# mcbuehler/DeepSEE

Hardware: AMD Instinct MI355X
Metric: train-step images/sec (G+D fwd+bwd), 8x 32->256 bs=8 (higher is better)
Workload: dtype fp32

## Files before the change

deepsee_amd/ops.py:

```python
import os
import ctypes as C

import threading

import torch

from . import lib as L
from .plan import KernelPlan, DEFAULT_PLAN, current as P

LRELU_SLOPE = 0.2
BN_EPS = 1e-5
BN_MOMENTUM = 0.1
SN_EPS = 1e-12
NHIDDEN = 128

_scratch = {}

PROFILE = None
PROFILE_BYTES = {}
PROFILE_OPERAND_GB = 0.0


def _variant(geom, modulate=False):
    halo = (geom.korder == 1 and geom.KH == 3 and geom.KW == 3 and geom.mul == 1 and geom.Hi == geom.Ho
# ... 1199 lines not shown
            dw = new(c)
            L.call("channel_dot_rng", dy, dw, C.c_long(m), c, ws, C.c_uint64(ctx.philox.seed),
                   C.c_uint64(ctx.philox.offset))
        elif eps is not None and ctx.needs_input_grad[1]:
            dw = channel_dot(dy, eps, c).clone()
        return dx, dw, None, None, None


class SeanInput(torch.autograd.Function):

    @staticmethod
    def forward(ctx, w_sh, b_sh, style, labels, shift, want_actv, want_style):
        n, h, w, nc = labels.n, labels.h, labels.w, labels.nc
        r, rw = h >> shift, w >> shift
        ld = (NHIDDEN if want_actv else 0) + (style.shape[2] if want_style else 0)
        cat = new(n, r, rw, ld)
        coff = 0
        if want_actv:
            table = new(9, nc, NHIDDEN)
            L.call("onehot_conv3x3_pack", w_sh.contiguous(), table, NHIDDEN, nc)
            L.call("onehot_conv3x3_fwd", labels.t, table, b_sh, cat, n, h, w, shift, nc, NHIDDEN, ld, 0, 1, -1, None, 0.0)
            coff = NHIDDEN
        if want_style:
            L.call("label_gather", labels.t, style.contiguous(), cat, n, h, w, shift, nc, style.shape[2], ld, coff, 1.0)
        ctx.labels, ctx.shift, ctx.want_actv, ctx.want_style, ctx.coff = labels, shift, want_actv, want_style, coff
        ctx.sshape = style.shape if want_style else None
        ctx.save_for_backward(cat)
        return cat

    @staticmethod
    def backward(ctx, dcat):
        (cat,) = ctx.saved_tensors
        lab, shift = ctx.labels, ctx.shift
        dcat = dcat.contiguous()
        n, r, rw, ld = cat.shape
        dw = db = dstyle = None
        if ctx.want_actv and ctx.needs_input_grad[0]:
            dw, db = new(NHIDDEN, lab.nc, 3, 3), new(NHIDDEN)
            ws = scratch(L.lib().dsee_onehot_conv3x3_wgrad_workspace(n, lab.h, lab.w, shift, lab.nc), "ohw")
            L.call("onehot_conv3x3_wgrad", lab.t, dcat, ld, cat, ld, n, lab.h, lab.w, shift, lab.nc, dw, db, ws)
        if ctx.want_style and ctx.needs_input_grad[2]:
            s = ctx.sshape[2]
            dstyle = new(*ctx.sshape)
            ws = scratch(L.lib().dsee_label_segsum_workspace(n, lab.h, lab.w, shift, lab.nc, s), "seg")
            L.call("label_segsum", lab.t, dcat, ld, ctx.coff, dstyle, n, lab.h, lab.w, shift, lab.nc, s, 1.0, ws)
        return dw, db, dstyle, None, None, None, None


class StylePool(torch.autograd.Function):

    @staticmethod
    def forward(ctx, feat, labels, shift):
        n, hf, wf, c = feat.shape
        assert hf == labels.h >> shift
        out = new(n, labels.nc, c)
        ws = scratch(L.lib().dsee_label_segsum_workspace(n, labels.h, labels.w, shift, labels.nc, c), "seg")
        L.call("label_segsum", labels.t, feat, c, 0, out, n, labels.h, labels.w, shift, labels.nc, c,
               1.0 / (hf * wf), ws)
        ctx.labels, ctx.shift, ctx.fshape = labels, shift, feat.shape
        return out

    @staticmethod
    def backward(ctx, ds):
        lab = ctx.labels
        n, hf, wf, c = ctx.fshape
        df = new(*ctx.fshape)
        L.call("label_gather", lab.t, ds.contiguous(), df, n, lab.h, lab.w, ctx.shift, lab.nc, c, c, 0, 1.0 / (hf * wf))
        return df, None, None


_perm_cache = {}


def packed_perm(c, device):
    key = (c, str(device))
    if key not in _perm_cache:
        rows = (c + 63) // 64 * 128
        idx = torch.full((rows,), 2 * c, dtype=torch.long)
        for p in range(rows):
            b, rem = divmod(p, 128)
            w, rem = divmod(rem, 64)
            h, cc = divmod(rem, 32)
            ch = b * 64 + w * 32 + cc
            if ch < c:
                idx[p] = h * c + ch
        _perm_cache[key] = (idx.to(device), rows)
    return _perm_cache[key]


def pack_gamma_beta(w_gamma, w_beta, b_gamma, b_beta):
    c = w_gamma.shape[0]
    idx, rows = packed_perm(c, w_gamma.device)
    zw = torch.zeros((1,) + tuple(w_gamma.shape[1:]), dtype=w_gamma.dtype, device=w_gamma.device)
    zb = torch.zeros(1, dtype=w_gamma.dtype, device=w_gamma.device)
    w2 = torch.cat([w_gamma, w_beta, zw], 0).index_select(0, idx)
    b2 = torch.cat([b_gamma, b_beta, zb], 0).index_select(0, idx)
    return w2, b2


class SeanPack(torch.autograd.Function):

    @staticmethod
    def forward(ctx, mode, wg, wb, wsg, wsb, bg, bb, bsg, bsb, ag, ab, amax=None):
        ref = wg if wg is not None else wsg
        c = ref.shape[0]
        k = wg.shape[1] if wg is not None else 0
        sdim = wsg.shape[1] if wsg is not None else 0
        rows = L.lib().dsee_sean_pack_rows(c)
        w2a = new(rows, k, 3, 3) if mode != 2 else None
        wst = new(9 * rows, sdim) if mode in (1, 2) else None
        b2 = new(rows)
        L.call("sean_pack_fwd", wg, wb, wsg, wsb, bg, bb, bsg, bsb, ag, ab, int(mode), c, k, sdim, w2a, wst, b2, amax)
        ctx.mode, ctx.dims = int(mode), (c, k, sdim, rows)
        ctx.save_for_backward(wg, wb, wsg, wsb, bg, bb, bsg, bsb, ag, ab)
        return w2a, wst, b2

    @staticmethod
    def backward(ctx, dw2a, dwst, db2):
        wg, wb, wsg, wsb, bg, bb, bsg, bsb, ag, ab = ctx.saved_tensors
        c, k, sdim, rows = ctx.dims
        mode = ctx.mode
        if mode != 2 and dw2a is None:
            dw2a = torch.zeros(rows, k, 3, 3, dtype=torch.float32, device=db2.device if db2 is not None else wg.device)
        if mode in (1, 2) and dwst is None:
            dwst = torch.zeros(9 * rows, sdim, dtype=torch.float32, device=wsg.device)
        outs = [torch.empty_like(t) if (t is not None and ctx.needs_input_grad[i + 1]) else None
                for i, t in enumerate((wg, wb, wsg, wsb, bg, bb, bsg, bsb))]
        dalpha = new(2) if (mode in (1, 3) and (ctx.needs_input_grad[9] or ctx.needs_input_grad[10])) else None
        ws = scratch(L.lib().dsee_sean_pack_bwd_workspace(), "seanpack")
        L.call("sean_pack_bwd", wg, wb, wsg, wsb, bg, bb, bsg, bsb, ag, ab, mode, c, k, sdim,
               None if dw2a is None else dw2a.contiguous(), None if dwst is None else dwst.contiguous(),
               None if db2 is None else db2.contiguous(), *outs, dalpha, ws)
        da = (dalpha[0:1], dalpha[1:2]) if dalpha is not None else (None, None)
        return (None, *outs, da[0] if ctx.needs_input_grad[9] else None, da[1] if ctx.needs_input_grad[10] else None, None)


class TableLayout(torch.autograd.Function):

    @staticmethod
    def forward(ctx, t, n, nc, rows, amax=None):
        ctx.dims = (n, nc, rows)
        out = new(n, 9, rows, 32)
        L.call("style_table_layout", t.contiguous(), out, n, nc, rows, amax)
        return out

    @staticmethod
    def backward(ctx, dout):
        n, nc, rows = ctx.dims
        dt = new(n * nc, 9 * rows)
        L.call("style_table_layout_bwd", dout.contiguous(), dt, n, nc, rows)
        return dt, None, None, None, None


def style_table_packed(style, wst, rows, amax=None):
    n, nc, s = style.shape
    t = TableLayout.apply(_style_gemm(style.reshape(n * nc, s), wst), n, nc, rows, amax)
    t.dsee_amax = amax
    return t


class SyncBNConfig:

    def __init__(self, world, group=None, clamp=True):
        self.world, self.group, self.clamp = int(world), group, bool(clamp)


def _stats_rows_ok(c):
    return P().sync_bn is None and c % 4 == 0 and c // 4 <= 256 and 256 % (c // 4) == 0


def bn_stats(x, running_mean, running_var, training):
    n, h, w, c = x.shape
    mean, invstd = new(c), new(c)
    if not training:
        L.call("norm_eval_stats", running_mean, running_var, c, BN_EPS, mean, invstd)
        return mean, invstd, None
    cfg = P().sync_bn
    if cfg is None:
        rows = getattr(x, "dsee_stats_rows", None)
        if rows is not None:
            L.call("norm_stats_finalize_parts", rows[0], rows[1], c, BN_EPS, BN_MOMENTUM, mean, invstd, running_mean,
                   running_var)
            return mean, invstd, None
        part = getattr(x, "dsee_stats_part", None)
        if part is None:
            part = torch.empty(L.lib().dsee_norm_workspace(n, h * w, c, 1) // 4, dtype=torch.float32, device="cuda")
            L.call("norm_stats_partial", x, n, h * w, c, 1, part)
            if P().share_stats:
                x.dsee_stats_part = part
        L.call("norm_stats_finalize", part, n, h * w, c, 1, BN_EPS, BN_MOMENTUM, mean, invstd, running_mean, running_var)
        return mean, invstd, None
    ws = scratch(L.lib().dsee_norm_workspace(n, h * w, c, 1), "norm")
    from . import parallel
    local = new(2, c)
    L.call("norm_stats_local", x, n, h * w, c, local, ws)
    rows = parallel.gather_stats(local, cfg.world, cfg.group)
    L.call("norm_stats_merge", rows, cfg.world, n * h * w, c, BN_EPS, BN_MOMENTUM, int(cfg.clamp), mean, invstd,
           running_mean, running_var)
    return mean, invstd, cfg


def in_stats(x):
    n, h, w, c = x.shape
    mean, invstd = new(n, c), new(n, c)
    part = getattr(x, "dsee_in_part", None)
    if part is None:
        part = torch.empty(L.lib().dsee_norm_workspace(n, h * w, c, n) // 4, dtype=torch.float32, device="cuda")
        L.call("norm_stats_partial", x, n, h * w, c, n, part)
        if P().share_stats:
            x.dsee_in_part = part
    L.call("norm_stats_finalize", part, n, h * w, c, n, BN_EPS, BN_MOMENTUM, mean, invstd, None, None)
    return mean, invstd


def norm_stats(x, running_mean, running_var, training):
    if running_mean is None:
        mean, invstd = in_stats(x)
        return mean, invstd, None
    return bn_stats(x, running_mean, running_var, training)


def stat_groups(mean):
    return mean.shape[0] if mean.dim() == 2 else 1


def _call_sg(name, sg, head, tail):
    if sg == 1:
        L.call(name, *head, *tail)
    else:
        L.call(name + "_sg", *head, sg, *tail)


def _wino_ws(n, h, w, c, sg):
    return (L.lib().dsee_modulate_bwd_wino_workspace(n, h, w, c) if sg == 1
            else L.lib().dsee_modulate_bwd_wino_workspace_sg(n, h, w, c, sg))


def modulate_bwd(dh, out, x, scale, mean, invstd, rows, cfg, as_dm=False, add=None, xhat_amax=None, mask=None):
    n, h, w, c = x.shape
    sg = stat_groups(mean)
    dx = torch.empty_like(x)
    sums = new(2 * sg + 2, c)
    dgb = dm = None
    t = n * (h // 4) * (w // 4)
    dha = carried_amax(dh)
    pre = (as_dm and P().presplit_dm and P().presplit_gb and xhat_amax is not None and dha is not None and t % 256 == 0
           and sg == 1)
    s16 = scale.dtype == torch.float16
    if s16 and not (pre and P().half):
        scale, s16 = scale.float(), False
    if pre:
        ga = amax_slot()
        L.call("amax_product", dha, xhat_amax, 1.0, ga)
        pk = P().half
        dm = (_i16(36 * t * rows * (1 if pk else 2)), ga, "pk" if pk else True)
        ws = scratch(L.lib().dsee_modulate_bwd_wino_workspace(n, h, w, c), "norm")
        L.call("modulate_bwd_reduce_wino_f16p" if pk else "modulate_bwd_reduce_wino_f16x2", dh.contiguous(),
               None if mask is not None else out, x, scale, mean, invstd, dm[0], rows, sums, n, h, w, c, LRELU_SLOPE, ws, ga,
               DM_BOUND, mask)
    elif as_dm:
        dm = (new(36, t, rows), amax_slot() if (P().gemm_split and (P().gemm_f16x2 or P().half)) else None)
        ws = scratch(_wino_ws(n, h, w, c, sg), "norm")
        _call_sg("modulate_bwd_reduce_wino", sg, (dh.contiguous(), out, x, scale, mean, invstd, dm[0], rows, sums, n, h, w, c),
                 (LRELU_SLOPE, ws, dm[1]))
    else:
        dgb = (torch.zeros if c % 64 else torch.empty)(n, h, w, rows, dtype=torch.float32, device=x.device)
        ws = scratch(L.lib().dsee_norm_workspace(n, h * w, c, sg), "norm")
        _call_sg("modulate_bwd_reduce", sg, (dh.contiguous(), out, x, scale, mean, invstd, dgb, rows, sums, n, h * w, c),
                 (LRELU_SLOPE, ws))
    count = (n // sg) * h * w
    if cfg is not None:
        from . import parallel
        parallel.allreduce_sums(sums[0:2], cfg.world, cfg.group)
        count *= cfg.world
    da = amax_slot()
    _call_sg("modulate_bwd_apply_amax", sg,
             (dh.contiguous(), None if mask is not None else out, x, scale, mean, invstd, sums, add, dx, n, h * w, c),
             (1.0 / count, LRELU_SLOPE, da, int(s16), mask))
    tag_amax(dx, da)
    return dx, dgb, sums[2 * sg:2 * sg + 2], dm


class SpadeNormAct(torch.autograd.Function):

    @staticmethod
    def forward(ctx, x, cat, w2, b2, running_mean, running_var, training, add_one, cat_ups, grad_sink=None):
        ctx.plan = P()
        ctx.grad_sink = grad_sink
        n, h, w, c = x.shape
        rows, kin = w2.shape[0], w2.shape[1]
        assert cat.shape[3] == kin and kin % 4 == 0
        mean, invstd, ctx.sync = norm_stats(x, running_mean, running_var, training)
        geom = L.geom_fwd(n, cat.shape[1], cat.shape[2], kin, rows, 3, 1, 1, cat_ups)
        assert geom.Ho == h and geom.Wo == w
        w2 = w2.contiguous()
        out, scale = torch.empty_like(x), torch.empty_like(x)
        wp = _pack_fwd(w2, kin, geom.korder)
        with _timed(_variant(geom, True), _flops(geom)):
            _call_sg("conv2d_modulate_fwd", stat_groups(mean),
                     (C.byref(geom), cat, wp, None, 0, b2.contiguous(), x, mean, invstd, out, scale, c),
                     (float(add_one), LRELU_SLOPE))
        ctx.geom = geom
        ctx.save_for_backward(x, cat, w2, out, scale, mean, invstd)
        return out

    @staticmethod
    @_under_plan
    def backward(ctx, dh):
        x, cat, w2, out, scale, mean, invstd = ctx.saved_tensors
# ... 402 lines not shown
```

deepsee_amd/plan.py:

```python
import contextlib
import dataclasses
import threading
from typing import Any, Optional


@dataclasses.dataclass(frozen=True)
class KernelPlan:
    winograd: bool = True
    winograd_wgrad: bool = True
    winograd_mod: bool = True
    gemm_split: bool = True
    gemm_af32: bool = True
    keep_v: bool = True
    gemm_f16x2: bool = True
    half: bool = False
    half_norms: bool = True
    presplit_a: bool = True
    gemm_w4: bool = True
    dgrad_s2_parity: bool = True
    presplit_min_tiles: int = 512
    conv_halo_f16: bool = True
    onehot_wgrad_mfma: bool = True
    conv_amax_out: bool = True
    presplit_dm: bool = True
    presplit_gb: bool = True
    dout_sums: bool = True
    adjoint_dgrad: bool = True
    fuse_noise: bool = True
    thin_gemm: bool = True
    share_stats: bool = True
    producer_stats: bool = True
    fuse_dm: bool = True
    fused_norm: bool = True
    fused_w4: bool = False
    sign_mask: bool = True
    defer_act: bool = True
    branch_streams: bool = False
    conv_f16x2_min_flop: float = 1e9
    sync_bn: Optional[Any] = None

    def replace(self, **changes):
        return dataclasses.replace(self, **changes)

    @contextlib.contextmanager
    def active(self):
        prev = getattr(_tls, "plan", None)
        _tls.plan = self
        try:
            yield self
        finally:
            _tls.plan = prev

    @classmethod
    def fields(cls):
        return [f.name for f in dataclasses.fields(cls)]


def _env_overrides():
    import ast
    import os
    text = os.environ.get("DSEE_PLAN", "").strip()
    if not text:
        return {}
    out = {}
    for item in text.split(","):
        k, _, v = item.partition("=")
        k = k.strip()
        if k not in KernelPlan.fields():
            raise ValueError("DSEE_PLAN: unknown KernelPlan field %r (fields: %s)" % (k, ", ".join(KernelPlan.fields())))
        out[k] = ast.literal_eval(v.strip())
    return out


DEFAULT_PLAN = KernelPlan(**_env_overrides())
_tls = threading.local()


def current():
    return getattr(_tls, "plan", None) or DEFAULT_PLAN


def from_opt(opt):
    prec = getattr(opt, "precision", "fp32")
    if prec not in ("fp32", "fp16"):
        raise ValueError("opt.precision must be 'fp32' or 'fp16', got %r" % (prec,))
    over = getattr(opt, "kernel_plan", None)
    if isinstance(over, KernelPlan):
        plan = over
    else:
        plan = DEFAULT_PLAN.replace(**dict(over or {}))
    return plan.replace(half=(prec == "fp16"))
```

include/deepsee_hip.h:

```cpp
#ifndef DEEPSEE_HIP_H
#define DEEPSEE_HIP_H

#include <stddef.h>
#include <stdint.h>

#ifdef __cplusplus
extern "C" {
#endif

#ifndef __HIP_INCLUDE_HIP_HIP_RUNTIME_API_H__
typedef struct ihipStream_t* hipStream_t;
#endif

#define DSEE_OK 0
#define DSEE_EINVAL (-1)
#define DSEE_ELAUNCH (-2)
#define DSEE_EUNSUPPORTED (-3)

#define DSEE_ACT_NONE 0
#define DSEE_ACT_LRELU 1
#define DSEE_ACT_RELU 2
#define DSEE_ACT_TANH 3
#define DSEE_ACT_MASK 4

// ... 195 lines not shown
int dsee_norm_eval_stats(const float* running_mean, const float* running_var, int C, float eps, float* mean,
                         float* invstd, hipStream_t stream);
int dsee_norm_act_fwd(const float* x, const float* mean, const float* invstd, float* y, int N, int HW, int C,
                      int groups, int act, float slope, hipStream_t stream);
int dsee_norm_act_bwd(const float* dy, const float* y, const float* x, const float* mean, const float* invstd,
                      float* dx, int N, int HW, int C, int groups, int act, float slope, float* workspace,
                      hipStream_t stream);
int dsee_norm_act_fwd_amax(const float* x, const float* mean, const float* invstd, float* y, int N, int HW, int C,
                           int groups, int act, float slope, float* amax_y, hipStream_t stream);
int dsee_norm_act_bwd_amax(const float* dy, const float* y, const float* x, const float* mean, const float* invstd,
                           float* dx, int N, int HW, int C, int groups, int act, float slope, float* workspace,
                           float* amax_dx, hipStream_t stream);
int dsee_bn_act_fwd(const float* x, const float* mean, const float* invstd, const float* gamma, const float* beta, float* y,
                    int N, int HW, int C, int act, float slope, float* amax_y, hipStream_t stream);
int dsee_bn_act_bwd_reduce(const float* dy, const float* y, const float* x, const float* mean, const float* invstd, int N,
                           int HW, int C, int act, float slope, float* sums, float* workspace, hipStream_t stream);
int dsee_bn_act_bwd_apply(const float* dy, const float* y, const float* x, const float* mean, const float* invstd,
                          const float* gamma, const float* sums, const float* local_sums, float inv_count, float* dx,
                          float* dgamma, float* dbeta, int N, int HW, int C, int act, float slope, float* amax_dx,
                          hipStream_t stream);
int dsee_counter_inc(int64_t* counter, hipStream_t stream);
int dsee_modulate_bwd(const float* dh, const float* h, const float* x, const float* scale, const float* mean,
                      const float* invstd, const float* add, float* dx, float* dgb, int dgb_ld, float* col_sums, int N,
                      int HW, int C, float slope, float* workspace, hipStream_t stream);

int dsee_modulate_bwd_reduce(const float* dh, const float* h, const float* x, const float* scale, const float* mean,
                             const float* invstd, float* dgb, int dgb_ld, float* sums, int N, int HW, int C, float slope,
                             float* workspace, hipStream_t stream);
size_t dsee_modulate_bwd_wino_workspace(int N, int H, int W, int C);
int dsee_modulate_bwd_reduce_wino(const float* dh, const float* h, const float* x, const float* scale, const float* mean,
                                  const float* invstd, float* dM, int rows, float* sums, int N, int H, int W, int C,
                                  float slope, float* workspace, float* amax, hipStream_t stream);
int dsee_modulate_bwd_reduce_wino_f16x2(const float* dh, const float* h, const float* x, const float* scale,
                                        const float* mean, const float* invstd, void* dM2, int rows, float* sums, int N,
                                        int H, int W, int C, float slope, float* workspace, const float* amax_g, float bound,
                                        const uint32_t* sign_mask,
        hipStream_t stream);
int dsee_amax_product(const float* a, const float* b, float floor_b, float* out, hipStream_t stream);
int dsee_wino43_input_adjoint_amax(const float* dV, float* dx, int N, int H, int W, int C, float* amax_dx, hipStream_t stream);
int dsee_modulate_bwd_apply(const float* dh, const float* h, const float* x, const float* scale, const float* mean,
                            const float* invstd, const float* sums, const float* add, float* dx, int N, int HW, int C,
                            float inv_count, float slope, hipStream_t stream);
int dsee_modulate_bwd_apply_amax(const float* dh, const float* h, const float* x, const float* scale, const float* mean,
                                 const float* invstd, const float* sums, const float* add, float* dx, int N, int HW, int C,
                                 float inv_count, float slope, float* amax_dx, int scale_f16, const uint32_t* sign_mask,
        hipStream_t stream);

int dsee_spade_fused_fwd_sg(const void* V2, const void* U2, const float* amax_cat, float v_bound, const float* amax_u,
                            const float* bias_packed, const float* x, const float* mean, const float* invstd, float* out_h,
                            float* out_scale, int N, int H, int W, int C, int rows, int K, int groups, int stat_groups,
                            float add_one, float slope, float* amax_h, float* amax_xhat, uint32_t* sign_mask,
                            hipStream_t stream);
int dsee_spade_fused_fwd_f16p_sg(const void* V1, const void* U1, const float* amax_cat, float v_bound, const float* amax_u,
                                 const float* bias_packed, const float* x, const float* mean, const float* invstd,
                                 float* out_h, float* out_scale, int N, int H, int W, int C, int rows, int K, int groups,
                                 int stat_groups, float add_one, float slope, float* amax_h, float* amax_xhat,
                                 uint32_t* sign_mask, hipStream_t stream);
int dsee_wino43_output_modulate_sg(const float* M, const float* bias_packed, const float* x, const float* mean,
                                   const float* invstd, float* out_h, float* out_scale, int N, int H, int W, int C, int rows,
                                   int stat_groups, float add_one, float slope, const float* mscale, hipStream_t stream);
int dsee_conv2d_modulate_fwd_sg(const dsee_conv_geom* g, const float* in, const float* w_packed,
                                const float* style_table, int shared_cin, const float* bias_packed, const float* x,
                                const float* mean, const float* invstd, float* out_h, float* out_scale, int C,
                                int stat_groups, float add_one, float slope, hipStream_t stream);
int dsee_modulate_bwd_reduce_sg(const float* dh, const float* h, const float* x, const float* scale, const float* mean,
                                const float* invstd, float* dgb, int dgb_ld, float* sums, int N, int HW, int C,
                                int stat_groups, float slope, float* workspace, hipStream_t stream);
size_t dsee_modulate_bwd_wino_workspace_sg(int N, int H, int W, int C, int stat_groups);
int dsee_modulate_bwd_reduce_wino_sg(const float* dh, const float* h, const float* x, const float* scale,
                                     const float* mean, const float* invstd, float* dM, int rows, float* sums, int N, int H,
                                     int W, int C, int stat_groups, float slope, float* workspace, float* amax,
                                     hipStream_t stream);
int dsee_modulate_bwd_apply_amax_sg(const float* dh, const float* h, const float* x, const float* scale, const float* mean,
                                    const float* invstd, const float* sums, const float* add, float* dx, int N, int HW, int C,
                                    int stat_groups, float inv_count, float slope, float* amax_dx, int scale_f16,
                                    const uint32_t* sign_mask, hipStream_t stream);

int dsee_onehot_conv3x3_pack(const float* w_oihw, float* table, int Co, int L, hipStream_t stream);
int dsee_onehot_conv3x3_fwd(const uint8_t* lab, const float* table, const float* bias, float* out, int N, int H, int W,
                            int shift, int L, int Co, int out_ld, int coff, int relu, int onehot_coff, float* amax,
                            float amax_floor, hipStream_t stream);
size_t dsee_onehot_conv3x3_wgrad_workspace(int N, int H, int W, int shift, int L);
int dsee_onehot_conv3x3_wgrad(const uint8_t* lab, const float* dact, int dact_ld, const float* act, int act_ld, int N,
                              int H, int W, int shift, int L, float* dw_oihw, float* dbias, float* workspace,
                              hipStream_t stream);
int dsee_label_onehot(const uint8_t* lab, float* out, int N, int H, int W, int shift, int out_ld, int coff,
                      hipStream_t stream);
int dsee_label_gather(const uint8_t* lab, const float* table, float* out, int N, int H, int W, int shift, int L, int Cs,
                      int out_ld, int coff, float scale, hipStream_t stream);
size_t dsee_label_segsum_workspace(int N, int H, int W, int shift, int L, int Cs);
int dsee_label_segsum(const uint8_t* lab, const float* in, int ld, int coff, float* table, int N, int H, int W,
                      int shift, int L, int Cs, float scale, float* workspace, hipStream_t stream);

int dsee_upsample_noise_fwd(const float* x, const float* eps, const float* noise_w, float* y, int N, int H, int W, int C,
                            int ups, hipStream_t stream);
int dsee_upsample_noise_rng_fwd(const float* x, const float* noise_w, float* y, int N, int H, int W, int C, int ups,
                                uint64_t seed, uint64_t offset, hipStream_t stream);
int dsee_upsample_noise_rng_fwd_stats(const float* x, const float* noise_w, float* y, int N, int H, int W, int C, int ups,
                                      uint64_t seed, uint64_t offset, float* stats_part, hipStream_t stream);
int dsee_channel_dot_rng(const float* a, float* out, long M, int C, float* workspace, uint64_t seed, uint64_t offset,
                         hipStream_t stream);
int dsee_sumpool(const float* dy, float* dx, int N, int H, int W, int C, int ups, hipStream_t stream);
int dsee_sumpool_amax(const float* dy, float* dx, int N, int H, int W, int C, int ups, float* amax_dx, hipStream_t stream);
size_t dsee_sumpool_dot_rng_workspace(int N, int H, int W, int C, int ups);
int dsee_sumpool_dot_rng(const float* dy, float* dx, int N, int H, int W, int C, int ups, float* amax_dx, float* dnoise_w,
                         float* workspace, uint64_t seed, uint64_t offset, hipStream_t stream);
size_t dsee_channel_dot_workspace(long M, int C);
int dsee_channel_dot(const float* a, const float* b, float* out, long M, int C, float* workspace, hipStream_t stream);
int dsee_act_fwd(const float* x, float* y, long n, int act, float slope, hipStream_t stream);
int dsee_act_bwd(const float* dy, const float* y, float* dx, long n, int act, float slope, hipStream_t stream);
int dsee_act_bwd_amax(const float* dy, const float* y, float* dx, long n, int act, float slope, float* amax_dx,
                      hipStream_t stream);
int dsee_axpby(const float* a, float alpha, const float* b, float beta, float* y, long n, hipStream_t stream);
int dsee_avgpool3s2_fwd(const float* x, float* y, int N, int H, int W, int C, hipStream_t stream);
int dsee_avgpool3s2_bwd(const float* dy, float* dx, int N, int H, int W, int C, hipStream_t stream);
int dsee_maxpool2_fwd(const float* x, float* y, int N, int H, int W, int C, hipStream_t stream);
int dsee_maxpool2_bwd(const float* dy, const float* x, float* dx, int N, int H, int W, int C, hipStream_t stream);
int dsee_nchw_to_nhwc(const float* x, float* y, int N, int C, int H, int W, int Cs, hipStream_t stream);
int dsee_nhwc_to_nchw(const float* x, float* y, int N, int C, int H, int W, int Cs, hipStream_t stream);
int dsee_label_to_u8(const float* label, uint8_t* out, long n, hipStream_t stream);
int dsee_bicubic_down(const float* x, float* y, int N, int H, int W, int S, int cs_in, int cs_out, hipStream_t stream);
int dsee_image_u8_to_nhwc(const uint8_t* img, const uint8_t* flip, float* out, int N, int H, int W, int cs_out,
                          hipStream_t stream);
int dsee_label_u8_prepare(const uint8_t* lab, const uint8_t* flip, uint8_t* out, int N, int H, int W, int unknown_to,
                          hipStream_t stream);
int dsee_build_d_input(const uint8_t* lab, const float* img, float* out, long pixels, int L, int Cs, int img_cs,
                       hipStream_t stream);
int dsee_build_d_input_amax(const uint8_t* lab, const float* img, float* out, long pixels, int L, int Cs, int img_cs,
                            float* amax_out, hipStream_t stream);
int dsee_extract_image_grad(const float* din, float* dimg, long pixels, int L, int Cs, int img_cs, hipStream_t stream);
int dsee_rng_fill(float* out, long n, uint64_t seed, uint64_t offset, int normal, hipStream_t stream);
int dsee_rng_set_epoch(const uint64_t* epoch_dev);

size_t dsee_loss_workspace(void);
int dsee_loss_fwd_bwd(int mode, const float* a, const float* b, float* grad, long rows, int ld, int valid_c,
                      float weight, float* loss_out, float* workspace, hipStream_t stream);
int dsee_loss_bwd(int mode, const float* a, const float* b, float* grad, long rows, int ld, int valid_c, float weight,
                  const float* upstream, hipStream_t stream);

int dsee_sean_pack_rows(int C);
int dsee_sean_pack_fwd(const float* w_gamma, const float* w_beta, const float* ws_gamma, const float* ws_beta,
                       const float* b_gamma, const float* b_beta, const float* bs_gamma, const float* bs_beta,
                       const float* alpha_gamma, const float* alpha_beta, int mode, int C, int K, int S, float* w2a,
                       float* wst, float* b2, float* amax_w2a, hipStream_t stream);
size_t dsee_sean_pack_bwd_workspace(void);
int dsee_sean_pack_bwd(const float* w_gamma, const float* w_beta, const float* ws_gamma, const float* ws_beta,
                       const float* b_gamma, const float* b_beta, const float* bs_gamma, const float* bs_beta,
                       const float* alpha_gamma, const float* alpha_beta, int mode, int C, int K, int S,
                       const float* dw2a, const float* dwst, const float* db2, float* dw_gamma, float* dw_beta,
                       float* dws_gamma, float* dws_beta, float* db_gamma, float* db_beta, float* dbs_gamma,
                       float* dbs_beta, float* dalpha, float* workspace, hipStream_t stream);
int dsee_style_table_layout(const float* t, float* table, int N, int L, int rows, float* amax, hipStream_t stream);
int dsee_style_table_layout_bwd(const float* dtable, float* dt, int N, int L, int rows, hipStream_t stream);

int dsee_spectral_norm_fwd(const float* w_orig, float* u, float* v, float* sigma, float* w_sn, int R, int K,
                           int power_iter, float eps, float* scratch, hipStream_t stream);
int dsee_spectral_norm_bwd(const float* dw, const float* w_sn, const float* u, const float* v, const float* sigma,
                           float* dw_orig, int R, int K, float* scratch, hipStream_t stream);

typedef struct dsee_sn_layer {
  const float* w_orig;
  float* u;
  float* v;
  int64_t out_off;
  int64_t saved_off;
  int32_t R, K;
  int32_t scratch_off;
  int32_t pad_;
} dsee_sn_layer;
int dsee_spectral_norm_group_fwd(const dsee_sn_layer* layers, int nlayers, const int* work_k, int n_k, const int* work_r,
                                 int n_r, const int* work_e, int n_e, int power_iter, float eps, float* scratch,
                                 float* sigma, float* out, float* saved, float* amax, hipStream_t stream);

typedef struct dsee_adam_tensor {
  int64_t offset;
  int64_t numel;
  int32_t first_block;
  int32_t step;
  float lr;
  int32_t active;
} dsee_adam_tensor;
int dsee_adam_step(float* param, const float* grad, float* exp_avg, float* exp_avg_sq,
                   const dsee_adam_tensor* tensors, const int* block_tensor, int nblocks, float beta1, float beta2,
                   float eps, float grad_scale, float clip, hipStream_t stream);
int dsee_grad_gather(const int64_t* grad_ptrs, const dsee_adam_tensor* tensors, const int* block_tensor, int nblocks,
                     float* grad_flat, int* active, hipStream_t stream);
int dsee_adam_step_range(float* param, const float* grad, float* exp_avg, float* exp_avg_sq,
                         const dsee_adam_tensor* tensors, const int* block_tensor, int first_block, int nblocks,
                         float beta1, float beta2, float eps, float grad_scale, float clip, hipStream_t stream);

#define DSEE_COMM_ID_BYTES 128
int dsee_comm_unique_id(void* id_out);
int dsee_comm_init(void** comm_out, const void* id, int world, int rank);
int dsee_comm_world(const void* comm);
int dsee_comm_rank(const void* comm);
int dsee_comm_allreduce_sum(void* comm, float* buf, long n, hipStream_t stream);
int dsee_comm_broadcast(void* comm, void* buf, long nbytes, int root, hipStream_t stream);
int dsee_comm_allgather(void* comm, const void* send, void* recv, long nbytes_per_rank, hipStream_t stream);
int dsee_comm_destroy(void* comm);

size_t dsee_sean_norm_fwd_workspace(int N, int H, int W, int C, int label_nc, int has_table);
int dsee_sean_norm_fwd(const uint8_t* labels, int lab_h, int lab_w, int shift, int label_nc, const float* w_shared,
                       const float* b_shared, const float* w2a, const float* table, const float* bias_packed, const float* x,
                       float* running_mean, float* running_var, int training, float eps, float momentum, float add_one,
                       float slope, float* out_h, float* out_scale, uint32_t* sign_mask, float* mean, float* invstd,
                       float* amax_h, int N, int H, int W, int C, void* workspace, size_t workspace_bytes,
                       hipStream_t stream);

typedef struct dsee_norm_layer {
  const float* w_shared;
  const float* b_shared;
  const float* w2a;
  const float* table;
  const float* bias_packed;
  float* running_mean;
  float* running_var;
  float add_one;
} dsee_norm_layer;
size_t dsee_spade_resblock_fwd_workspace(int N, int H, int W, int C, int label_nc, int has_table);
int dsee_spade_resblock_fwd(const dsee_norm_layer* norm_0, const float* w_conv_0, const float* b_conv_0,
                            const dsee_norm_layer* norm_1, const float* w_conv_1, const float* b_conv_1,
                            const uint8_t* labels, int lab_h, int lab_w, int shift, int label_nc, const float* x, float* out,
                            int out_act, int training, float eps, float momentum, float slope, int N, int H, int W, int C,
                            void* workspace, size_t workspace_bytes, hipStream_t stream);

typedef struct dsee_block_noise {
  const float* w_middle;
  uint64_t seed_middle, offset_middle;
  const float* w_skip;
  uint64_t seed_skip, offset_skip;
} dsee_block_noise;
typedef struct dsee_norm_grads {
  float* dw_shared;
  float* db_shared;
  float* dw2a;
  float* dtable;
  float* dgamma_beta_sums;
} dsee_norm_grads;
typedef struct dsee_block_grads {
  dsee_norm_grads norm_0, norm_1;
  float* dw_conv_0;
  float* db_conv_0;
  float* dw_conv_1;
  float* db_conv_1;
  float* dw_noise_middle;
  float* dw_noise_skip;
} dsee_block_grads;
size_t dsee_spade_resblock_saved_bytes(int N, int H, int W, int C, int label_nc, int has_table);
size_t dsee_spade_resblock_train_fwd_workspace(int N, int H, int W, int C, int label_nc, int has_table);
int dsee_spade_resblock_train_fwd(const dsee_norm_layer* norm_0, const float* w_conv_0, const float* b_conv_0,
                                  const dsee_norm_layer* norm_1, const float* w_conv_1, const float* b_conv_1,
                                  const dsee_block_noise* noise, const uint8_t* labels, int lab_h, int lab_w, int shift,
                                  int label_nc, const float* x, float* out, float eps, float momentum, float slope, int N, int H,
                                  int W, int C, void* saved, size_t saved_bytes, void* workspace, size_t workspace_bytes,
                                  hipStream_t stream);
size_t dsee_spade_resblock_bwd_workspace(int N, int H, int W, int C, int label_nc, int has_table, int lab_h, int lab_w, int shift);
int dsee_spade_resblock_bwd(const dsee_norm_layer* norm_0, const float* w_conv_0, const dsee_norm_layer* norm_1,
                            const float* w_conv_1, const dsee_block_noise* noise, const uint8_t* labels, int lab_h, int lab_w,
                            int shift, int label_nc, const float* x, const float* dout, const float* amax_dout,
                            const dsee_block_grads* grads, float* dx, float* amax_dx, float slope, int N, int H, int W, int C,
                            const void* saved, size_t saved_bytes, void* workspace, size_t workspace_bytes, hipStream_t stream);

#ifdef __cplusplus
}
#endif
#endif
```

Baseline: 92.05.

## Fuse style-table GEMM and table layout into one MFMA kernel

Adds a dedicated HIP kernel that computes the style projection directly into the packed per-sample table layout, replacing a generic GEMM followed by a separate layout kernel. The backward pass computes the weight gradient and a split-K style gradient in one launch, then reduces the splits in a finalize kernel. The aim is to drop the intermediate buffer, an extra launch and a layout pass in both directions. In exchange it adds a workspace for the partial sums and a shape-restricted path (S multiple of 32 and at most 256, at most 32 classes) that falls back to the old route otherwise.

New measurement: 92.25, median of 6. No clear change (+0.2%).

```diff
diff --git a/deepsee_amd/csrc/style_table.hip b/deepsee_amd/csrc/style_table.hip
--- /dev/null
+++ b/deepsee_amd/csrc/style_table.hip
@@ -0,0 +1,164 @@
+#include "dsee_common.h"
+
+namespace {
+
+constexpr int ST_JT = 32;
+constexpr int ST_JS = 144;
+constexpr int ST_SMAX = 256;
+
+__device__ __forceinline__ f32x16 st_mfma(float a, float b, const f32x16& c) {
+  return __builtin_amdgcn_mfma_f32_32x32x2f32(a, b, c, 0, 0, 0);
+}
+__device__ __forceinline__ int st_row(int v, int h) { return (v & 3) + 8 * (v >> 2) + 4 * h; }
+
+__global__ __launch_bounds__(256) void style_table_fwd_kernel(const float* __restrict__ style, const float* __restrict__ wst,
+                                                              float* __restrict__ table, int N, int L, int S, int J,
+                                                              float* __restrict__ amax) {
+  __shared__ __attribute__((aligned(16))) float a_lds[ST_JT * (ST_SMAX + 4)];
+  const int j0 = blockIdx.x * ST_JT, ld = S + 4, s4 = S >> 2;
+  for (int i = threadIdx.x; i < ST_JT * s4; i += 256) {
+    const int row = i / s4, c4 = i - row * s4;
+    *reinterpret_cast<f32x4*>(a_lds + row * ld + 4 * c4) =
+        *reinterpret_cast<const f32x4*>(wst + (size_t)(j0 + row) * S + 4 * c4);
+  }
+  __syncthreads();
+  const int lane = threadIdx.x & 63, wave = threadIdx.x >> 6, col = lane & 31, h = lane >> 5;
+  const int sh = S >> 1;
+  const bool live = col < L;
+  const float* ap = a_lds + col * ld + h * sh;
+  float vmax = 0.f;
+  for (int n = wave; n < N; n += 4) {
+    const float* bp = style + ((size_t)n * L + (live ? col : 0)) * S + h * sh;
+    f32x16 acc0 = {0}, acc1 = {0};
+    f32x4 a0 = *reinterpret_cast<const f32x4*>(ap), a1 = *reinterpret_cast<const f32x4*>(ap + 4);
+    f32x4 b0 = *reinterpret_cast<const f32x4*>(bp), b1 = *reinterpret_cast<const f32x4*>(bp + 4);
+    for (int q = 0; q < sh; q += 8) {
+      const int qn = q + 8 < sh ? q + 8 : q;
+      const f32x4 na0 = *reinterpret_cast<const f32x4*>(ap + qn), na1 = *reinterpret_cast<const f32x4*>(ap + qn + 4);
+      const f32x4 nb0 = *reinterpret_cast<const f32x4*>(bp + qn), nb1 = *reinterpret_cast<const f32x4*>(bp + qn + 4);
+      if (!live) b0 = b1 = f32x4{0.f, 0.f, 0.f, 0.f};
+#pragma unroll
+      for (int e = 0; e < 4; ++e) {
+        acc0 = st_mfma(a0[e], b0[e], acc0);
+        acc1 = st_mfma(a1[e], b1[e], acc1);
+      }
+      a0 = na0, a1 = na1, b0 = nb0, b1 = nb1;
+    }
+    float* op = table + ((size_t)n * J + j0) * 32 + col;
+#pragma unroll
+    for (int v = 0; v < 16; ++v) {
+      const float x = live ? acc0[v] + acc1[v] : 0.f;
+      op[(size_t)st_row(v, h) * 32] = x;
+      vmax = fmaxf(vmax, fabsf(x));
+    }
+  }
+  if (amax) dsee_block_atomic_absmax(amax, vmax);
+}
+
+__global__ __launch_bounds__(256) void style_table_bwd_kernel(const float* __restrict__ dT, const float* __restrict__ style,
+                                                              const float* __restrict__ wst, float* __restrict__ dwst,
+                                                              float* __restrict__ partial, int N, int L, int S, int J,
+                                                              int nb_w) {
+  const int lane = threadIdx.x & 63, wave = threadIdx.x >> 6, col = lane & 31, h = lane >> 5;
+  if ((int)blockIdx.x < nb_w) {
+    const int j0 = blockIdx.x * ST_JT, Lh = (L + 1) >> 1;
+    for (int s0 = wave * 32; s0 < S; s0 += 128) {
+      f32x16 acc0 = {0}, acc1 = {0};
+      for (int n = 0; n < N; ++n) {
+        const float* ap = dT + ((size_t)n * J + j0 + col) * 32;
+        const float* bp = style + (size_t)n * L * S + s0 + col;
+        const int r0 = h * Lh < L ? h * Lh : L - 1;
+        float a = ap[r0], b = bp[(size_t)r0 * S];
+        for (int t = 0; t < Lh; ++t) {
+          const bool ok = h * Lh + t < L;
+          const int rn = h * Lh + t + 1 < L ? h * Lh + t + 1 : L - 1;
+          const float na = ap[rn], nb = bp[(size_t)rn * S];
+          if (!ok) a = b = 0.f;
+          if (t & 1) acc1 = st_mfma(a, b, acc1);
+          else acc0 = st_mfma(a, b, acc0);
+          a = na, b = nb;
+        }
+      }
+      float* op = dwst + (size_t)j0 * S + s0 + col;
+#pragma unroll
+      for (int v = 0; v < 16; ++v) op[(size_t)st_row(v, h) * S] = acc0[v] + acc1[v];
+    }
+    return;
+  }
+  const int b2 = blockIdx.x - nb_w, n = b2 % N, sp = b2 / N;
+  const int jb = sp * ST_JS + h * (ST_JS / 2);
+  const bool live = col < L;
+  for (int s0 = wave * 32; s0 < S; s0 += 128) {
+    f32x16 acc0 = {0}, acc1 = {0};
+#pragma unroll 8
+    for (int t = 0; t < ST_JS / 2; ++t) {
+      const int j = jb + t;
+      const bool ok = j < J;
+      const int jj = ok ? j : J - 1;
+      float a = dT[((size_t)n * J + jj) * 32 + col], b = wst[(size_t)jj * S + s0 + col];
+      if (!(ok && live)) a = 0.f;
+      if (!ok) b = 0.f;
+      if (t & 1) acc1 = st_mfma(a, b, acc1);
+      else acc0 = st_mfma(a, b, acc0);
+    }
+    float* op = partial + ((size_t)sp * N + n) * L * S + s0 + col;
+#pragma unroll
+    for (int v = 0; v < 16; ++v) {
+      const int r = st_row(v, h);
+      if (r < L) op[(size_t)r * S] = acc0[v] + acc1[v];
+    }
+  }
+}
+
+__global__ __launch_bounds__(256) void style_table_bwd_finalize_kernel(const float* __restrict__ partial,
+                                                                       float* __restrict__ dstyle, int total, int nsplit) {
+  __shared__ float red[4][64];
+  const int o = threadIdx.x & 63, g = threadIdx.x >> 6, i = blockIdx.x * 64 + o;
+  const int q = (nsplit + 3) >> 2, lo = g * q, hi = min(nsplit, lo + q);
+  float s = 0.f;
+  if (i < total) {
+#pragma unroll 8
+    for (int sp = lo; sp < hi; ++sp) s += partial[(size_t)sp * total + i];
+  }
+  red[g][o] = s;
+  __syncthreads();
+  if (g == 0 && i < total) dstyle[i] = ((red[0][o] + red[1][o]) + red[2][o]) + red[3][o];
+}
+
+inline int st_splits(int J) { return (J + ST_JS - 1) / ST_JS; }
+inline bool st_shape_ok(int N, int L, int S, int rows) {
+  return N > 0 && L > 0 && L <= 32 && S > 0 && S % 32 == 0 && S <= ST_SMAX && rows > 0 && (9 * rows) % ST_JT == 0;
+}
+
+}
+
+extern "C" {
+
+int dsee_style_table_fwd(const float* style, const float* wst, float* table, int N, int L, int S, int rows, float* amax,
+                         hipStream_t st) {
+  DSEE_CHECK_ARG(style && wst && table && st_shape_ok(N, L, S, rows));
+  const int J = 9 * rows;
+  style_table_fwd_kernel<<<J / ST_JT, 256, 0, st>>>(style, wst, table, N, L, S, J, amax);
+  DSEE_LAUNCH_CHECK();
+  return DSEE_OK;
+}
+
+size_t dsee_style_table_bwd_workspace(int N, int L, int S, int rows) {
+  return (size_t)st_splits(9 * rows) * N * L * S * sizeof(float);
+}
+
+int dsee_style_table_bwd(const float* dtable, const float* style, const float* wst, float* dstyle, float* dwst, int N, int L,
+                         int S, int rows, float* workspace, hipStream_t st) {
+  DSEE_CHECK_ARG(dtable && style && wst && st_shape_ok(N, L, S, rows) && (!dstyle || workspace));
+  const int J = 9 * rows, nb_w = dwst ? J / ST_JT : 0, nsplit = st_splits(J), nb_s = dstyle ? nsplit * N : 0;
+  if (nb_w + nb_s == 0) return DSEE_OK;
+  style_table_bwd_kernel<<<nb_w + nb_s, 256, 0, st>>>(dtable, style, wst, dwst, workspace, N, L, S, J, nb_w);
+  if (dstyle) {
+    const int total = N * L * S;
+    style_table_bwd_finalize_kernel<<<(total + 63) / 64, 256, 0, st>>>(workspace, dstyle, total, nsplit);
+  }
+  DSEE_LAUNCH_CHECK();
+  return DSEE_OK;
+}
+
+}
diff --git a/deepsee_amd/ops.py b/deepsee_amd/ops.py
--- a/deepsee_amd/ops.py
+++ b/deepsee_amd/ops.py
@@ -1375,9 +1375,35 @@
         return dt, None, None, None, None
 
 
+class StyleTable(torch.autograd.Function):
+
+    @staticmethod
+    def forward(ctx, style, wst, rows, amax=None):
+        n, nc, s = style.shape
+        style, wst = style.contiguous(), wst.contiguous()
+        out = new(n, 9, rows, 32)
+        L.call("style_table_fwd", style, wst, out, n, nc, s, rows, amax)
+        ctx.save_for_backward(style, wst)
+        ctx.rows = rows
+        return out
+
+    @staticmethod
+    def backward(ctx, dout):
+        style, wst = ctx.saved_tensors
+        n, nc, s = style.shape
+        dstyle = torch.empty_like(style) if ctx.needs_input_grad[0] else None
+        dwst = torch.empty_like(wst) if ctx.needs_input_grad[1] else None
+        ws = scratch(L.lib().dsee_style_table_bwd_workspace(n, nc, s, ctx.rows), "styletab")
+        L.call("style_table_bwd", dout.contiguous(), style, wst, dstyle, dwst, n, nc, s, ctx.rows, ws)
+        return dstyle, dwst, None, None
+
+
 def style_table_packed(style, wst, rows, amax=None):
     n, nc, s = style.shape
-    t = TableLayout.apply(_style_gemm(style.reshape(n * nc, s), wst), n, nc, rows, amax)
+    if P().style_table_kernel and s % 32 == 0 and s <= 256 and nc <= 32:
+        t = StyleTable.apply(style, wst, rows, amax)
+    else:
+        t = TableLayout.apply(_style_gemm(style.reshape(n * nc, s), wst), n, nc, rows, amax)
     t.dsee_amax = amax
     return t
 
diff --git a/deepsee_amd/plan.py b/deepsee_amd/plan.py
--- a/deepsee_amd/plan.py
+++ b/deepsee_amd/plan.py
@@ -36,6 +36,7 @@
     sign_mask: bool = True
     defer_act: bool = True
     branch_streams: bool = False
+    style_table_kernel: bool = True
     conv_f16x2_min_flop: float = 1e9
     sync_bn: Optional[Any] = None
 
diff --git a/include/deepsee_hip.h b/include/deepsee_hip.h
--- a/include/deepsee_hip.h
+++ b/include/deepsee_hip.h
@@ -371,6 +371,11 @@
                        float* dbs_beta, float* dalpha, float* workspace, hipStream_t stream);
 int dsee_style_table_layout(const float* t, float* table, int N, int L, int rows, float* amax, hipStream_t stream);
 int dsee_style_table_layout_bwd(const float* dtable, float* dt, int N, int L, int rows, hipStream_t stream);
+int dsee_style_table_fwd(const float* style, const float* wst, float* table, int N, int L, int S, int rows, float* amax,
+                         hipStream_t stream);
+size_t dsee_style_table_bwd_workspace(int N, int L, int S, int rows);
+int dsee_style_table_bwd(const float* dtable, const float* style, const float* wst, float* dstyle, float* dwst, int N, int L,
+                         int S, int rows, float* workspace, hipStream_t stream);
 
 int dsee_spectral_norm_fwd(const float* w_orig, float* u, float* v, float* sigma, float* w_sn, int R, int K,
                            int power_iter, float eps, float* scratch, hipStream_t stream);
```
